# jabirali/bodge

Measured on AMD Instinct MI355X. Metric: Chebyshev SpMV steps/s + achieved HBM GB/s, 4N×4N BdG H; free_energy wall-time, higher is better.
Workload: dtype f64

## Files before the change

### bodge_amd/backend.py

```python

from __future__ import annotations

import ctypes as C
import os

import numpy as np

LIBRARY_PATH = os.environ.get(
    "BODGE_AMD_LIBRARY", os.path.join(os.path.dirname(os.path.abspath(__file__)), "csrc", "libbodge_hip.so")
)

VEC_RADEMACHER = 0
VEC_Z4 = 1

_f64p = C.POINTER(C.c_double)
_i32p = C.POINTER(C.c_int32)
_i64p = C.POINTER(C.c_int64)
_u8p = C.POINTER(C.c_uint8)
_handle = C.c_void_p


class Perf(C.Structure):
    _fields_ = [
        ("kernel_ms", C.c_double),
# ... 18 lines not shown
        ("window_ms", C.c_double),
        ("sweeps", C.c_int64),
        ("persistent", C.c_int32),
        ("groups_per_launch", C.c_int32),
        ("clenshaw", C.c_int32),
        ("green", C.c_int32),
        ("green_ranges", C.c_int32),
        ("green_local", C.c_int32),
        ("apply", C.c_int32),
        ("green_states", C.c_int32),
        ("green_bonds", C.c_int32),
        ("roll_chunk", C.c_int32),
        ("response_map", C.c_int32),
        ("gemm_ms", C.c_double),
        ("gemm_flops", C.c_double),
        ("correlation", C.c_int32),
        ("gram_ms", C.c_double),
        ("gram_flops", C.c_double),
    ]


class Operator(C.Structure):

    _fields_ = [("nnzb", C.c_int32), ("indptr", _i32p), ("indices", _i32p), ("data", _f64p)]


SIGNATURES = {
    "bdg_last_error": (C.c_char_p, []),
    "bdg_version": (C.c_char_p, []),
    "bdg_device_count": (C.c_int, [C.POINTER(C.c_int)]),
# ... 167 lines not shown
```

### bodge_amd/build.py

```python

from __future__ import annotations

import os
import shutil
import subprocess
import sys

ROOT = os.path.dirname(os.path.abspath(__file__))
CSRC = os.path.join(ROOT, "csrc")
INCLUDE = os.path.join(os.path.dirname(ROOT), "include")
LIBRARY = os.path.join(CSRC, "libbodge_hip.so")
SOURCES = [os.path.join(CSRC, "bodge_hip.hip")]
HEADERS = [os.path.join(CSRC, name) for name in (
    "kernels.hpp", "sweep.hpp", "twostage.hpp", "host_assembly.hpp", "core.hpp", "plans.hpp", "libraries.hpp", "recurrence.hpp", "family.hpp", "fermi.hpp", "apply.hpp", "correlation.hpp", "response_map.hpp", "green_driver.hpp", "green.hpp", "green_map.hpp", "green_bonds.hpp", "green_states.hpp",
    "lanczos.hpp", "subspace.hpp", "dense.hpp", "tridiag.hpp", "knobs.hpp")] + [os.path.join(INCLUDE, "bodge_hip.h")]
ARCH = "gfx950"


def _hipcc() -> str:
    found = shutil.which("hipcc") or "/opt/rocm/bin/hipcc"
    if not os.path.exists(found):
        raise RuntimeError("hipcc not found; the HIP library cannot be built")
    return found


def is_stale() -> bool:
    if not os.path.exists(LIBRARY):
        return True
    built = os.path.getmtime(LIBRARY)
# ... 27 lines not shown
```

### bodge_amd/csrc/bodge_hip.hip

```cpp

#include "bodge_hip.h"

#include <dlfcn.h>
#include <fcntl.h>
#include <hip/hip_runtime.h>
#include <rccl/rccl.h>
#include <rocsolver/rocsolver.h>

#include <sys/stat.h>
#include <unistd.h>

#include <algorithm>
#include <atomic>
#include <chrono>
#include <condition_variable>
#include <cmath>
#include <cstdarg>
#include <cstdio>
#include <cstdlib>
#include <cstring>
#include <map>
#include <memory>
#include <mutex>
#include <string>
#include <string_view>
#include <thread>
#include <tuple>
#include <type_traits>
#include <unordered_map>
#include <vector>

#include "knobs.hpp"
#include "host_assembly.hpp"
#include "kernels.hpp"
#include "sweep.hpp"
#include "twostage.hpp"

#include "core.hpp"
#include "plans.hpp"
#include "libraries.hpp"
#include "recurrence.hpp"
#include "family.hpp"
#include "fermi.hpp"
#include "apply.hpp"
#include "correlation.hpp"
#include "response_map.hpp"
#include "green_driver.hpp"
#include "green.hpp"
#include "green_map.hpp"
#include "green_bonds.hpp"
// ... 48 lines not shown
                return fail(BDG_EINVAL, "column index %d out of range in row %lld", indices[k],
                            (long long)i);
            if (k > indptr[i] && indices[k] == indices[k - 1])
                return fail(BDG_EINVAL, "row %lld has a duplicate column", (long long)i);
            if (ncols == nb && k > indptr[i] && indices[k] < indices[k - 1])
                return fail(BDG_EINVAL, "row %lld is not sorted", (long long)i);
            bandwidth = std::max<int64_t>(bandwidth, std::llabs((long long)indices[k] - (long long)i));
        }
    }
    constexpr int kMaxDistinct = 256;
    constexpr unsigned kStreamedId = 0xFEu;
    int dict_skipped = 0;
    bool onsite_streamed = false, bonds_streamed = false;
    std::vector<int> ids;
    std::vector<double> distinct;
    {
        const char* env = knob::raw("BODGE_AMD_DICT");
        bool wanted = !(env && env[0] == '0') && nnzb > 0 && ncols <= (1 << 24);
        dict_skipped = (env && env[0] == '0') ? 3 : ncols > (1 << 24) ? 2 : 0;
        auto onsite_packable = [](const double* blk) {
            auto re = [&](int r, int c) { return blk[2 * (4 * r + c)]; };
            auto im = [&](int r, int c) { return blk[2 * (4 * r + c) + 1]; };
            if (im(0, 0) != 0.0 || im(1, 1) != 0.0 || re(1, 0) != re(0, 1) || im(1, 0) != -im(0, 1)) return false;
            for (int i = 0; i < 2; ++i)
                for (int j = 0; j < 2; ++j) {
                    if (re(2 + i, j) != re(j, 2 + i) || im(2 + i, j) != -im(j, 2 + i)) return false;
                    if (re(2 + i, 2 + j) != -re(i, j) || im(2 + i, 2 + j) != im(i, j)) return false;
                }
            return true;
        };
        auto dedupe = [&](bool skip_diagonal, int limit) -> bool {
            std::unordered_map<std::string_view, int> seen;
            const double* recent_key[4] = {nullptr, nullptr, nullptr, nullptr};
            int recent_id[4] = {0, 0, 0, 0};
            int recent_next = 0;
            ids.assign((size_t)nnzb, 0);
            distinct.clear();
            for (int64_t i = 0; i < nb; ++i)
                for (int64_t k = indptr[i]; k < indptr[i + 1]; ++k) {
                    const double* block = data + 32 * k;
                    if (skip_diagonal && indices[k] == i) {
                        if (!onsite_packable(block)) return false;
                        ids[(size_t)k] = (int)((unsigned)indices[k] | (kStreamedId << 24));
                        continue;
                    }
// ... 168 lines not shown
    if (!ids.empty()) {
        sys->n_unique = (int)(distinct.size() / 32);
        if (int rc = sys->dict_ids.reserve(ids.size())) return cleanup(rc);
        if (int rc = sys->dict_full.reserve((size_t)sys->n_unique * 16)) return cleanup(rc);
        std::vector<int> diagonal((size_t)sys->n_unique, 1);
        for (int d = 0; d < sys->n_unique; ++d)
            for (int e = 0; e < 16; ++e)
                if ((e >> 2) != (e & 3) && (distinct[(size_t)32 * d + 2 * e] != 0.0 || distinct[(size_t)32 * d + 2 * e + 1] != 0.0))
                    diagonal[(size_t)d] = 0;
        for (int d = 0; d < sys->n_unique; ++d) {
            if (diagonal[(size_t)d]) continue;
            auto zero = [&](int r, int c) { return distinct[(size_t)32 * d + 2 * (4 * r + c)] == 0.0 && distinct[(size_t)32 * d + 2 * (4 * r + c) + 1] == 0.0; };
            if (zero(0, 1) && zero(1, 0) && zero(0, 2) && zero(1, 3) && zero(2, 0) && zero(3, 1) && zero(2, 3) && zero(3, 2)) diagonal[(size_t)d] = 2;
        }
        if (knob::raw("BODGE_AMD_NO_DIAGONAL_BLOCKS")) std::fill(diagonal.begin(), diagonal.end(), 0);
        if (int rc = sys->dict_diagonal.reserve((size_t)sys->n_unique)) return cleanup(rc);
        if (hipMemcpy(sys->dict_diagonal.ptr, diagonal.data(), sizeof(int) * diagonal.size(), hipMemcpyHostToDevice) != hipSuccess)
            return cleanup(fail(BDG_EDEVICE, "upload of the block dictionary failed"));
        if (!onsite_streamed && max_row <= 7) {
            const int words = max_row <= 3 ? 4 : 8;
            std::vector<unsigned> ell((size_t)nb * words, 0xFFFFFFFFu);
            for (int64_t i = 0; i < nb; ++i)
                for (int64_t k = indptr[i]; k < indptr[i + 1]; ++k) ell[(size_t)i * words + (size_t)(k - indptr[i])] = (unsigned)ids[(size_t)k];
            if (int rc = sys->dict_ell.reserve(ell.size())) return cleanup(rc);
            if (hipMemcpy(sys->dict_ell.ptr, ell.data(), sizeof(unsigned) * ell.size(), hipMemcpyHostToDevice) != hipSuccess)
                return cleanup(fail(BDG_EDEVICE, "upload of the block dictionary failed"));
            sys->dict_ell_words = words;
        }
        if (hipMemcpy(sys->dict_ids.ptr, ids.data(), sizeof(int) * ids.size(), hipMemcpyHostToDevice) != hipSuccess ||
            hipMemcpy(sys->dict_full.ptr, distinct.data(), sizeof(double) * distinct.size(),
// ... 780 lines not shown
```

### bodge_amd/csrc/core.hpp

```cpp
#pragma once

namespace {

thread_local std::string g_error;

int fail(int code, const char* fmt, ...) {
    char buf[512];
    va_list ap;
    va_start(ap, fmt);
    vsnprintf(buf, sizeof buf, fmt, ap);
    va_end(ap);
    g_error = buf;
    return code;
}

#define HIP_TRY(expr)                                                                   \
    do {                                                                                \
        hipError_t err__ = (expr);                                                      \
        if (err__ != hipSuccess)                                                        \
            return fail(err__ == hipErrorOutOfMemory ? BDG_ENOMEM : BDG_EDEVICE,        \
                        "%s failed: %s (%s:%d)", #expr, hipGetErrorString(err__),       \
                        __FILE__, __LINE__);                                            \
    } while (0)

// ... 138 lines not shown
    int dict_skipped = 0;
    bool onsite_streamed = false;
    DeviceBuffer<double2> onsite[2];
    bool bonds_streamed = false;
    DeviceBuffer<double2> site_records[2];
    int site_records_plane[2] = {0, 0};
    DeviceBuffer<int> dict_ids;
    DeviceBuffer<unsigned> dict_ell;
    int dict_ell_words = 0;
    DeviceBuffer<int> dict_diagonal;
    DeviceBuffer<double2> dict_full;
    DeviceBuffer<double2> dict_table[4];
    DeviceBuffer<uint2> stencil;
    int stencil_state = 0;
    bool stencil_wrap_p = false, stencil_wrap_x = false;
    double* host_dots = nullptr;
    size_t host_dots_count = 0;
    int shape[3] = {0, 0, 0};
    struct TileOrder {
        int rows_per_tile = 0, strip_rows = 0;
        DeviceBuffer<int> ids;
    };
    std::vector<std::unique_ptr<TileOrder>> tile_orders;
    bdg_perf perf{};
};

namespace {
inline void release_side_sets(bdg_system* sys) {
    for (auto& side : sys->side_sets) {
        if (side->stream) (void)hipStreamSynchronize(side->stream);
// ... 20 lines not shown
```

### bodge_amd/csrc/plans.hpp

```cpp
#pragma once

namespace {

using StepKernel = void (*)(bdg::StepArgs);

using bdg::ComplexMode;
using bdg::ComplexPHMode;
using bdg::RealMode;
using bdg::RealPHMode;

struct ModeInfo {
    int id;
    bool real, ph;
    int per_lane;
    int stride;
    double block_bytes;
    double entry_bytes;
};

ModeInfo mode_info(bool real, bool ph) {
    if (real && ph) return {3, true, true, RealPHMode::kVec, RealPHMode::kBlockStride, 100.0, 96.0};
    if (real) return {1, true, false, RealMode::kVec, RealMode::kBlockStride, 132.0, 96.0};
    if (ph) return {2, false, true, ComplexPHMode::kVec, ComplexPHMode::kBlockStride, 196.0, 192.0};
    return {0, false, false, ComplexMode::kVec, ComplexMode::kBlockStride, 260.0, 192.0};
// ... 441 lines not shown
        const int resident = waves * (int)std::min<size_t>(waves > 4 ? 1 : 2, sys->lds_per_cu / lds);
        if (resident > best_resident) best = waves, best_resident = resident;
    }
    return best;
}

SweepKernel sweep3_kernel(const ModeInfo& mode, int lanes, bool reverse) {
    switch (mode.id) {
        case 1: return sweep3_kernel_for<RealMode>(lanes, reverse);
        case 2: return sweep3_kernel_for<ComplexPHMode>(lanes, reverse);
        case 3: return sweep3_kernel_for<RealPHMode>(lanes, reverse);
    }
    return sweep3_kernel_for<ComplexMode>(lanes, reverse);
}

using MarchKernel = void (*)(bdg::MarchArgs);
template <typename Mode>
MarchKernel march3_kernel_for(int lanes) {
    switch (lanes) {
        case 2: return bdg::cheb_march3<Mode, 2, 0>;
        case 4: return bdg::cheb_march3<Mode, 4, 0>;
    }
    return nullptr;
}
MarchKernel march3_kernel(const ModeInfo& mode, int lanes, bool streamed, bool bonds) {
    if (streamed) {
        if (!mode.ph || lanes != 4) return nullptr;
        if (bonds) return mode.real ? bdg::cheb_march3<RealPHMode, 4, 2> : nullptr;
        return mode.real ? bdg::cheb_march3<RealPHMode, 4, 1> : bdg::cheb_march3<ComplexPHMode, 4, 1>;
    }
    switch (mode.id) {
        case 1: return march3_kernel_for<RealMode>(lanes);
        case 2: return march3_kernel_for<ComplexPHMode>(lanes);
        case 3: return march3_kernel_for<RealPHMode>(lanes);
    }
    return march3_kernel_for<ComplexMode>(lanes);
}

struct SweepPlan {
    int lanes = bdg::kSweepLanes;
    int depth = 2;
    SweepKernel kernel = nullptr, kernel_reverse = nullptr;
    SweepKernel kernel_gen = nullptr;
    MarchKernel march = nullptr;
    int march_grid = 0;
    int grid = 0;
    int wg_waves = bdg::kSweepWaves;
    size_t lds_bytes = 0;
    bdg::SweepArgs args{};
    int waves = 0;
    int whole_segs = 1;
    int segments_for(int planes) const {
        if (planes >= args.lx) return whole_segs;
        return std::max(1, std::min(choose_segments(args.n_cols, planes, waves, 2 * depth, 2), planes / 2));
    }
};

constexpr int64_t kSweepMinSites = 150000;
// ... 20 lines not shown
                if (x == 0 && (lo < 0 || lo == base)) lo = base;
                else if (x == lx - 1 && (hi < 0 || hi == base)) hi = base;
                else slab_ok = false;
            }
            for (int64_t base : {lo, hi})
                if (base >= 0 && (base < sys->nb || base + plane > sys->ncols)) slab_ok = false;
            if (slab_ok) {
                sys->stencil_lo_base = (int)lo;
                sys->stencil_hi_base = (int)hi;
            }
        }
        if (shaped && slab_ok && sys->n_unique > 0 && sys->n_unique < (int)bdg::kNoBlock &&
            sys->max_row_blocks <= (three_d ? 7 : 5) && sys->nnzb > 0 && !(three_d && sys->onsite_streamed)) {
            if (int rc = sys->stencil.reserve((size_t)sys->nb)) return rc;
            DeviceBuffer<int> bad;
            if (int rc = bad.reserve(3)) return rc;
            int host_bad[3] = {1, 0, 0};
            auto body = [&]() -> int {
                HIP_TRY(hipMemsetAsync(bad.ptr, 0, 3 * sizeof(int), sys->stream));
                const unsigned grid = (unsigned)std::min<int64_t>(4096, (sys->nb + 255) / 256);
                if (three_d)
                    bdg::build_stencil3<<<grid, 256, 0, sys->stream>>>(sys->indptr.ptr, sys->dict_ids.ptr,
                                                                        sys->dict_diagonal.ptr, (int)sys->nb, (int)plane,
                                                                        sys->shape[2], sys->stencil_lo_base, sys->stencil_hi_base,
                                                                        sys->stencil.ptr, bad.ptr);
                else
                    bdg::build_stencil<<<grid, 256, 0, sys->stream>>>(sys->indptr.ptr, sys->dict_ids.ptr,
                                                                       sys->dict_diagonal.ptr, (int)sys->nb, (int)plane,
                                                                       sys->bonds_streamed ? 2 : sys->onsite_streamed ? 1 : 0,
                                                                       sys->stencil.ptr, bad.ptr);
                HIP_TRY(hipGetLastError());
                HIP_TRY(hipMemcpyAsync(host_bad, bad.ptr, 3 * sizeof(int), hipMemcpyDeviceToHost, sys->stream));
                HIP_TRY(hipStreamSynchronize(sys->stream));
                return BDG_OK;
            };
            const int rc = body();
            bad.release();
            if (rc) return rc;
            if (host_bad[0] == 0) {
                sys->stencil_state = three_d ? 2 : 1;
                sys->stencil_wrap_p = host_bad[1] != 0;
                sys->stencil_wrap_x = host_bad[2] != 0;
            } else {
                sys->stencil.release();
            }
        }
    }
    *kind = std::max(0, sys->stencil_state);
    return BDG_OK;
}

inline int64_t plane_sites(const bdg_system* sys) { return (int64_t)sys->shape[1] * sys->shape[2]; }

int sweep_wanted(bdg_system* sys, bool col_scalars, int* kind, bool wide_call = false) {
    *kind = 0;
    const char* env = knob::raw("BODGE_AMD_SWEEP");
    if ((env && env[0] == '0') || col_scalars) return BDG_OK;
// ... 20 lines not shown
        return fail(BDG_EINVAL, "streamed on-site blocks need the three-step sweep, particle-hole packed blocks and a lane count whose ring of records fits the LDS (%d lanes do not)", lanes);
    plan->wg_waves = wg_waves;
    plan->kernel = streamed ? sweep3_streamed_kernel(mode, lanes, wg_waves, false, false, bonds)
                            : depth == 3 ? sweep3_kernel(mode, lanes, false) : sweep_kernel(mode, lanes, false);
    plan->kernel_reverse = streamed ? sweep3_streamed_kernel(mode, lanes, wg_waves, true, false, bonds)
                                    : depth == 3 ? sweep3_kernel(mode, lanes, true) : sweep_kernel(mode, lanes, true);
    plan->kernel_gen = streamed ? sweep3_streamed_kernel(mode, lanes, wg_waves, false, true, bonds) : depth == 3 ? sweep3_gen_kernel(mode, lanes) : nullptr;
    if (!plan->kernel) return fail(BDG_EINVAL, "the sweep kernel has 1, 2 or 4 lanes per site, not %d", lanes);
    const size_t table = (size_t)sys->n_unique * mode.stride * sizeof(double2);
    if (table > table_limit(sys)) return fail(BDG_EINVAL, "block table too large for the sweep kernel");
    if (depth == 3) {
        plan->lds_bytes = sweep3_lds_bytes(sys, mode, lanes, wg_waves);
    } else {
        plan->lds_bytes = table + (size_t)bdg::kSweepWaves * depth * bdg::kWave * 4 * sizeof(double2);
    }
    if (plan->lds_bytes > 64 * 1024)
        for (SweepKernel k : {plan->kernel, plan->kernel_reverse, plan->kernel_gen})
            if (k) HIP_TRY(hipFuncSetAttribute(reinterpret_cast<const void*>(k), hipFuncAttributeMaxDynamicSharedMemorySize,
                                        (int)plan->lds_bytes));
    plan->march = depth == 3 && wg_waves == bdg::kWavesPerBlock &&
                          (size_t)sys->ncols * lanes * 4 * sizeof(double2) < ((size_t)1 << 31) && sys->ncols == sys->nb
                      ? march3_kernel(mode, lanes, streamed, bonds) : nullptr;
    if (plan->march && plan->lds_bytes > 64 * 1024)
        HIP_TRY(hipFuncSetAttribute(reinterpret_cast<const void*>(plan->march), hipFuncAttributeMaxDynamicSharedMemorySize,
                                    (int)plan->lds_bytes));
    int per_cu = 0;
    HIP_TRY(hipOccupancyMaxActiveBlocksPerMultiprocessor(&per_cu, reinterpret_cast<const void*>(plan->kernel),
                                                         wg_waves * bdg::kWave, plan->lds_bytes));
    per_cu = std::max(1, std::min(per_cu, wg_waves > 4 ? 1 : 2 * bdg::kWavesPerBlock / bdg::kSweepWaves));
    if (const char* cap = knob::raw("BODGE_AMD_BLOCKS_PER_CU")) per_cu = std::max(1, atoi(cap));
    const int64_t plane = (int64_t)sys->shape[1] * sys->shape[2];
    bdg::SweepArgs& a = plan->args;
// ... 12 lines not shown
    const int owned = depth == 3 ? bdg::sweep3_owned(lanes) : bdg::sweep_owned(lanes);
    a.n_cols = (int)((plane + owned - 1) / owned);
    if (const char* env = knob::raw("BODGE_AMD_STREAMED_SHARE"); streamed && (wg_waves > 4 || (env && env[0] == '0'))) share = 1;
    const int waves = std::max(wg_waves, per_cu * sys->num_cus * wg_waves / std::max(1, share));
    int n_segs = choose_segments(a.n_cols, a.lx, waves, 2 * depth, 8, share > 1 ? 0.985 : 0.97);
    if (const char* env = knob::raw("BODGE_AMD_SWEEP_SEGMENTS")) n_segs = atoi(env);
    a.n_segs = std::max(1, std::min(n_segs, a.lx / 8));
    a.x_lo = 0;
    a.x_hi = a.lx;
    plan->waves = waves;
    plan->whole_segs = a.n_segs;
    a.zigzag = 1;
    if (const char* env = knob::raw("BODGE_AMD_SWEEP_ZIGZAG")) a.zigzag = atoi(env) != 0;
    a.wrap_p = sys->stencil_wrap_p ? 1 : 0;
    a.wrap_x = sys->stencil_wrap_x ? 1 : 0;
    const int64_t units = (int64_t)a.n_cols * a.n_segs;
    const int grid = (int)std::min<int64_t>((int64_t)per_cu * sys->num_cus, (units + wg_waves - 1) / wg_waves);
    plan->grid = std::max(8, (grid + 7) / 8 * 8);
    const int march_grid = (int)std::min<int64_t>((int64_t)per_cu * sys->num_cus,
                                                  (units * std::max(1, share) + wg_waves - 1) / wg_waves);
    plan->march_grid = std::max(8, (march_grid + 7) / 8 * 8);
    return BDG_OK;
}

double sweep_bytes(const bdg_system* sys, const ModeInfo& mode, int lanes) {
    const double onsite = !sys->onsite_streamed ? 0.0
                          : sys->bonds_streamed ? (mode.real ? 128.0 : 224.0)
                          : 16.0 * (mode.real ? RealPHMode::kOnsiteSlots : ComplexPHMode::kOnsiteSlots);
    return (8.0 + onsite) * (double)sys->nb + (mode.block_bytes - 4.0) * sys->n_unique +
           4.0 * (4.0 * lanes * sizeof(double2)) * (double)sys->nb;
// ... 165 lines not shown
```

### bodge_amd/csrc/recurrence.hpp

```cpp
#pragma once

namespace {

constexpr int kMarchAborted = -77;

struct Batch {
    bdg_system* sys = nullptr;
    StreamSet* ss = nullptr;
    int next = 0;
    int stream_share = 1;
    StepPlan plan;
    bdg::StepArgs args{};
    bool real = false;
    bool alternate = false;
    int64_t band_lo = -1, band_hi = -1;
    int plane_lo = -1, plane_hi = -1;
    ModeInfo mode{};
    int rl = 0, rv = 0, n_active = 0, n_steps = 0, chunk = 1, strip_rows = 0;
    size_t width = 0, per_step = 0, vec_count = 0;
    double scale = 1.0;
    double2* cur = nullptr;
    double2* prev = nullptr;
    float kernel_ms = 0.f;
    int n_chunks = 0;
    bool sweep = false, roll = false;
    bool gen_start = false;
    int slot = 0, n_slots = 1, ev_base = 0;
    size_t host_stride = 0;
    SweepPlan splan;
    RollPlan rplan;
    double2 *spare1 = nullptr, *spare2 = nullptr;
    const double2 *ext_lo = nullptr, *ext_hi = nullptr;
    int64_t ext_lo_site0 = 0, ext_lo_ld = 0, ext_hi_site0 = 0, ext_hi_ld = 0;
    int launch_grid = 0;
    bool discard_last = true;
    double bytes_moved = 0.0;
    bool march = false, march_follower = false;
    int march_levels = 0;
    bool march_fixed = false;
    int n_sweeps = 0;
    int64_t sweeps_counted = 0;
    hipStream_t work_stream = nullptr;
    double vector_bytes() const { return 4.0 * rl * sizeof(double2) * (double)sys->nb; }
    int n_launches = 0;

    int begin(bdg_system* system, double scale_in, int steps, int active, const StartSpec& start,
              int force_real , bool col_scalars = false, int set_index = 0) {
        sys = system;
        scale = scale_in;
        n_steps = steps;
        n_active = active;
// ... 61 lines not shown
            if (int rc = make_sweep_plan(sys, mode, rl, sweep_depth_for(sys, rl), &splan, stream_share)) return rc;
        } else if (roll) {
            plan = StepPlan{};
            plan.rl = rl;
            plan.mode = mode;
            plan.dictionary = true;
            args = bdg::StepArgs{};
            if (int rc = make_roll_plan(sys, mode, rl, &rplan)) return rc;
            rplan.share = stream_share;
        } else {
            if (int rc = make_plan(sys, rl, mode, &plan, col_scalars)) return rc;
            if (int rc = matrix_args(sys, plan, &args)) return rc;
        }
        launch_grid = sweep ? splan.grid : roll ? rplan.grid : plan.grid;
        n_launches = 0;
        n_sweeps = 0;
        sweeps_counted = 0;
        bytes_moved = 0.0;
        work_stream = ss->stream;
        march_follower = false;
        march = sweep && splan.depth == 3 && splan.march != nullptr && !sys->march_off && n_steps >= 4 &&
                start.kind == StartKind::Random;
        march_levels = 0;
        march_fixed = false;
        {
            const char* env = knob::raw("BODGE_AMD_MARCH");
            const int kind = env ? atoi(env) : 0;
            march = march && kind >= 1 && kind <= 3;
            march_levels = kind == 2 ? 1 : 0;
            march_fixed = kind == 3;
// ... 359 lines not shown
        }
        if (in_chunk == 0) HIP_TRY(hipEventRecord(ss->ev_pool[2 * (ev_base + chunk_id)], st));
        bdg::SweepArgs& a = splan.args;
        a.cur = cur;
        a.prev = n == 0 ? nullptr : prev;
        a.out1 = spare1;
        a.out2 = spare2;
        a.coef1 = (n == 0 ? 1.0 : 2.0) / scale;
        a.coef2 = 2.0 / scale;
        a.two = now >= 2 ? 1 : 0;
        a.steps = now;
        a.discard = discard_last && n + now == n_steps;
        a.partial1 = ss->partial.ptr + (size_t)in_chunk * per_step;
        a.partial2 = a.partial1 + per_step;
        a.partial3 = a.partial2 + per_step;
        const SweepKernel kernel = n == 0 && gen_start ? splan.kernel_gen
                                   : alternate && (n_launches & 1) ? splan.kernel_reverse : splan.kernel;
        if (n == 0 && gen_start) a.cur = nullptr;
        a.x_lo = 0;
        a.x_hi = a.lx;
        if (plane_lo >= 0) {
            a.x_lo = std::max(0, plane_lo - (n + now));
            a.x_hi = std::min(a.lx, plane_hi + n + now + 1);
        }
        a.n_segs = splan.segments_for(a.x_hi - a.x_lo);
        bytes_moved += (sweep_bytes(sys, mode, rl) -
                        vector_bytes() * ((n == 0 ? 1 : 0) + (n == 0 && gen_start ? 1 : 0) + (a.discard ? 2 : now == 1 ? 1 : 0))) *
                       ((double)(a.x_hi - a.x_lo) / a.lx);
        kernel<<<splan.grid, splan.wg_waves * bdg::kWave, splan.lds_bytes, st>>>(a);
        ++n_launches;
        double2* old_cur = cur;
        double2* old_prev = prev;
// ... 80 lines not shown
            for (int r = 0; r < n_active; ++r) {
                double& d = d_out[(size_t)n * ld + col0 + r];
                double& e = e_out[(size_t)n * ld + col0 + r];
                const double dv = host[(size_t)n * width + 2 * r], ev = host[(size_t)n * width + 2 * r + 1];
                d = accumulate ? d + dv : dv;
                e = accumulate ? e + ev : ev;
            }
        bdg_perf& p = sys->perf;
        if (first_batch) p = bdg_perf{};
        p.kernel_ms += kernel_ms;
        p.launches += sweep ? n_launches : n_steps;
        p.bytes_moved += bytes_moved;
        p.window_ms = p.kernel_ms;
        p.streams = 1;
        p.vector_steps += (int64_t)n_steps * n_active;
        p.bytes_per_launch = sweep  ? sweep_bytes(sys, mode, rl)
                             : roll ? roll_bytes(sys, mode, rl)
                                    : algorithmic_bytes(sys, rv, mode, plan.dictionary);
        p.steps_per_launch = sweep ? splan.depth : 1;
        p.persistent = march ? 1 : 0;
        p.sweeps += march ? sweeps_counted : sweep ? n_launches : 0;
        p.rolling = roll ? 1 : 0;
        p.roll_chunk = roll ? rplan.args.chunk : 0;
        p.dict_skipped = sys->dict_skipped;
        p.onsite_streamed = sweep && sys->onsite_streamed ? (sys->bonds_streamed ? 2 : 1) : 0;
        p.lanes_per_row = rl;
        p.vectors_per_launch = rv;
        p.real_arithmetic = real ? 1 : 0;
        p.ph_packed = mode.ph ? 1 : 0;
        p.dict_blocks = plan.dictionary ? sys->n_unique : 0;
// ... 464 lines not shown
```

### bodge_amd/csrc/sweep.hpp

```cpp
#pragma once

#include "kernels.hpp"

namespace bdg {

constexpr int kSweepLanes = 4;
constexpr int kSweepSlots = kWave / kSweepLanes;
constexpr int kSweepOwned = kSweepSlots - 4;
constexpr int sweep_owned(int rl) { return kWave / rl - 4; }
constexpr unsigned kNoBlock = 0xFFu;

struct SweepArgs {
    const uint2* stencil;
    const void* dict_table;
    int n_unique;
    const double2* onsite;
    const double2* cur;
    const double2* prev;
    double2* out1;
    double2* out2;
    double* partial1;
    double* partial2;
    double coef1, coef2;
    int nb;
// ... 1 lines not shown
    int lx;
    int n_cols;
    int n_segs;
    int two;
    int steps;
    double* partial3;
    int stream;
    int zigzag;
    int wrap_p;
    int wrap_x;
    uint64_t gen_seed, gen_first_id;
    int gen_kind;
    int gen_active;
    int discard;
    int x_lo, x_hi;
};

__global__ void build_stencil(const int* __restrict__ indptr, const int* __restrict__ words,
                              const int* __restrict__ diagonal, int nb, int plane, int onsite_streamed,
                              uint2* __restrict__ stencil, int* __restrict__ bad) {
    const int lx = nb / plane;
    for (int i = blockIdx.x * blockDim.x + threadIdx.x; i < nb; i += gridDim.x * blockDim.x) {
        unsigned id[5] = {kNoBlock, kNoBlock, kNoBlock, kNoBlock, kNoBlock};
        unsigned mask = 0;
        const int p = i % plane, x = i / plane;
        bool ok = true;
        for (int k = indptr[i]; k < indptr[i + 1]; ++k) {
            const unsigned w = (unsigned)words[k];
            const int off = (int)(w & 0xFFFFFFu) - i;
            int slot = -1;
// ... 1202 lines not shown
```

### include/bodge_hip.h

```cpp
#ifndef BODGE_HIP_H
#define BODGE_HIP_H

#include <stdint.h>

#ifdef __cplusplus
extern "C" {
#endif

#define BDG_OK 0
#define BDG_EINVAL (-1)
#define BDG_EDEVICE (-2)
#define BDG_ENOMEM (-3)
#define BDG_ELIBRARY (-4)

#define BDG_VEC_RADEMACHER 0
#define BDG_VEC_Z4 1

typedef struct bdg_system bdg_system;
typedef struct bdg_comm bdg_comm;
typedef struct bdg_group bdg_group;

typedef struct bdg_perf {
    double kernel_ms;
    int64_t launches;
// ... 17 lines not shown
    double window_ms;
    int64_t sweeps;
    int32_t persistent;
    int32_t groups_per_launch;
    int32_t clenshaw;
    int32_t green;
    int32_t green_ranges;
    int32_t green_local;
    int32_t apply;
    int32_t green_states;
    int32_t green_bonds;
    int32_t roll_chunk;
    int32_t response_map;
    double gemm_ms;
    double gemm_flops;
    int32_t correlation;
    double gram_ms;
    double gram_flops;
} bdg_perf;

const char* bdg_last_error(void);
const char* bdg_version(void);

int bdg_device_count(int* count);

int bdg_create(int device, int64_t nb, int64_t nnzb, const int32_t* indptr,
               const int32_t* indices, const double* data, bdg_system** out);
int bdg_destroy(bdg_system* sys);

int bdg_create_slab(int device, int64_t nb, int64_t ncols, int64_t nnzb, const int32_t* indptr,
// ... 122 lines not shown
```

Before: 110,600.

## Add translation-invariant sweep kernel holding stencil blocks in registers

Adds a classification pass that detects when every site in a 2D lattice uses the same bond and onsite blocks with no wrap-around. For that case it selects a specialised depth-3 sweep kernel that loads the five blocks once into registers instead of reading a per-site stencil and dictionary entries. The goal is to remove the per-site stencil reads and table lookups from the memory-bound Chebyshev SpMV. The cost is an extra classification kernel at setup and more register pressure, and the fast path applies only to uniform lattices.

```diff
diff --git a/bodge_amd/backend.py b/bodge_amd/backend.py
--- a/bodge_amd/backend.py
+++ b/bodge_amd/backend.py
@@ -56,6 +56,7 @@
         ("response_map", C.c_int32),
         ("gemm_ms", C.c_double),
         ("gemm_flops", C.c_double),
+        ("plain_stencil", C.c_int32),
         ("correlation", C.c_int32),
         ("gram_ms", C.c_double),
         ("gram_flops", C.c_double),
diff --git a/bodge_amd/build.py b/bodge_amd/build.py
--- a/bodge_amd/build.py
+++ b/bodge_amd/build.py
@@ -12,7 +12,7 @@
 LIBRARY = os.path.join(CSRC, "libbodge_hip.so")
 SOURCES = [os.path.join(CSRC, "bodge_hip.hip")]
 HEADERS = [os.path.join(CSRC, name) for name in (
-    "kernels.hpp", "sweep.hpp", "twostage.hpp", "host_assembly.hpp", "core.hpp", "plans.hpp", "libraries.hpp", "recurrence.hpp", "family.hpp", "fermi.hpp", "apply.hpp", "correlation.hpp", "response_map.hpp", "green_driver.hpp", "green.hpp", "green_map.hpp", "green_bonds.hpp", "green_states.hpp",
+    "kernels.hpp", "sweep.hpp", "sweep_plain.hpp", "twostage.hpp", "host_assembly.hpp", "core.hpp", "plans.hpp", "libraries.hpp", "recurrence.hpp", "family.hpp", "fermi.hpp", "apply.hpp", "correlation.hpp", "response_map.hpp", "green_driver.hpp", "green.hpp", "green_map.hpp", "green_bonds.hpp", "green_states.hpp",
     "lanczos.hpp", "subspace.hpp", "dense.hpp", "tridiag.hpp", "knobs.hpp")] + [os.path.join(INCLUDE, "bodge_hip.h")]
 ARCH = "gfx950"
 
diff --git a/bodge_amd/csrc/bodge_hip.hip b/bodge_amd/csrc/bodge_hip.hip
--- a/bodge_amd/csrc/bodge_hip.hip
+++ b/bodge_amd/csrc/bodge_hip.hip
@@ -34,6 +34,7 @@
 #include "host_assembly.hpp"
 #include "kernels.hpp"
 #include "sweep.hpp"
+#include "sweep_plain.hpp"
 #include "twostage.hpp"
 
 #include "core.hpp"
@@ -112,21 +113,21 @@
     bool onsite_streamed = false, bonds_streamed = false;
     std::vector<int> ids;
     std::vector<double> distinct;
+    auto onsite_packable = [](const double* blk) {
+        auto re = [&](int r, int c) { return blk[2 * (4 * r + c)]; };
+        auto im = [&](int r, int c) { return blk[2 * (4 * r + c) + 1]; };
+        if (im(0, 0) != 0.0 || im(1, 1) != 0.0 || re(1, 0) != re(0, 1) || im(1, 0) != -im(0, 1)) return false;
+        for (int i = 0; i < 2; ++i)
+            for (int j = 0; j < 2; ++j) {
+                if (re(2 + i, j) != re(j, 2 + i) || im(2 + i, j) != -im(j, 2 + i)) return false;
+                if (re(2 + i, 2 + j) != -re(i, j) || im(2 + i, 2 + j) != im(i, j)) return false;
+            }
+        return true;
+    };
     {
         const char* env = knob::raw("BODGE_AMD_DICT");
         bool wanted = !(env && env[0] == '0') && nnzb > 0 && ncols <= (1 << 24);
         dict_skipped = (env && env[0] == '0') ? 3 : ncols > (1 << 24) ? 2 : 0;
-        auto onsite_packable = [](const double* blk) {
-            auto re = [&](int r, int c) { return blk[2 * (4 * r + c)]; };
-            auto im = [&](int r, int c) { return blk[2 * (4 * r + c) + 1]; };
-            if (im(0, 0) != 0.0 || im(1, 1) != 0.0 || re(1, 0) != re(0, 1) || im(1, 0) != -im(0, 1)) return false;
-            for (int i = 0; i < 2; ++i)
-                for (int j = 0; j < 2; ++j) {
-                    if (re(2 + i, j) != re(j, 2 + i) || im(2 + i, j) != -im(j, 2 + i)) return false;
-                    if (re(2 + i, 2 + j) != -re(i, j) || im(2 + i, 2 + j) != im(i, j)) return false;
-                }
-            return true;
-        };
         auto dedupe = [&](bool skip_diagonal, int limit) -> bool {
             std::unordered_map<std::string_view, int> seen;
             const double* recent_key[4] = {nullptr, nullptr, nullptr, nullptr};
@@ -325,6 +326,8 @@
             if (zero(0, 1) && zero(1, 0) && zero(0, 2) && zero(1, 3) && zero(2, 0) && zero(3, 1) && zero(2, 3) && zero(3, 2)) diagonal[(size_t)d] = 2;
         }
         if (knob::raw("BODGE_AMD_NO_DIAGONAL_BLOCKS")) std::fill(diagonal.begin(), diagonal.end(), 0);
+        sys->dict_packable.resize((size_t)sys->n_unique);
+        for (int d = 0; d < sys->n_unique; ++d) sys->dict_packable[(size_t)d] = onsite_packable(distinct.data() + (size_t)32 * d) ? 1 : 0;
         if (int rc = sys->dict_diagonal.reserve((size_t)sys->n_unique)) return cleanup(rc);
         if (hipMemcpy(sys->dict_diagonal.ptr, diagonal.data(), sizeof(int) * diagonal.size(), hipMemcpyHostToDevice) != hipSuccess)
             return cleanup(fail(BDG_EDEVICE, "upload of the block dictionary failed"));
diff --git a/bodge_amd/csrc/core.hpp b/bodge_amd/csrc/core.hpp
--- a/bodge_amd/csrc/core.hpp
+++ b/bodge_amd/csrc/core.hpp
@@ -176,6 +176,10 @@
     DeviceBuffer<uint2> stencil;
     int stencil_state = 0;
     bool stencil_wrap_p = false, stencil_wrap_x = false;
+    bool plain_stencil = false;
+    unsigned plain_ids = 0, plain_meta = 0;
+    int plain_onsite_form = 0;
+    std::vector<unsigned char> dict_packable;
     double* host_dots = nullptr;
     size_t host_dots_count = 0;
     int shape[3] = {0, 0, 0};
diff --git a/bodge_amd/csrc/plans.hpp b/bodge_amd/csrc/plans.hpp
--- a/bodge_amd/csrc/plans.hpp
+++ b/bodge_amd/csrc/plans.hpp
@@ -479,6 +479,16 @@
     return sweep3_kernel_for<ComplexMode>(lanes, reverse);
 }
 
+constexpr bool kSweepPlainDefault = true;
+template <int OSF>
+SweepKernel sweep3_plain_pick(bool reverse, bool gen) {
+    return gen ? bdg::cheb_sweep3_plain<RealPHMode, false, true, OSF>
+               : reverse ? bdg::cheb_sweep3_plain<RealPHMode, true, false, OSF> : bdg::cheb_sweep3_plain<RealPHMode, false, false, OSF>;
+}
+SweepKernel sweep3_plain_kernel(int form, bool reverse, bool gen) {
+    return form == 1 ? sweep3_plain_pick<1>(reverse, gen) : sweep3_plain_pick<0>(reverse, gen);
+}
+
 using MarchKernel = void (*)(bdg::MarchArgs);
 template <typename Mode>
 MarchKernel march3_kernel_for(int lanes) {
@@ -507,6 +517,8 @@
     int depth = 2;
     SweepKernel kernel = nullptr, kernel_reverse = nullptr;
     SweepKernel kernel_gen = nullptr;
+    bool plain = false;
+    SweepKernel plain_kernel = nullptr, plain_reverse = nullptr, plain_gen = nullptr;
     MarchKernel march = nullptr;
     int march_grid = 0;
     int grid = 0;
@@ -557,10 +569,16 @@
             sys->max_row_blocks <= (three_d ? 7 : 5) && sys->nnzb > 0 && !(three_d && sys->onsite_streamed)) {
             if (int rc = sys->stencil.reserve((size_t)sys->nb)) return rc;
             DeviceBuffer<int> bad;
-            if (int rc = bad.reserve(3)) return rc;
-            int host_bad[3] = {1, 0, 0};
+            if (int rc = bad.reserve(3 + bdg::kPlainWords)) return rc;
+            int host_bad[3 + bdg::kPlainWords] = {1, 0, 0, 1};
+            const bool classify = !three_d && !sys->onsite_streamed && !sys->bonds_streamed;
             auto body = [&]() -> int {
-                HIP_TRY(hipMemsetAsync(bad.ptr, 0, 3 * sizeof(int), sys->stream));
+                {
+                    int init[3 + bdg::kPlainWords] = {0};
+                    for (int slot = 0; slot < 5; ++slot) init[3 + 1 + slot] = 0xFF;
+                    HIP_TRY(hipMemcpyAsync(bad.ptr, init, sizeof(init), hipMemcpyHostToDevice, sys->stream));
+                    HIP_TRY(hipStreamSynchronize(sys->stream));
+                }
                 const unsigned grid = (unsigned)std::min<int64_t>(4096, (sys->nb + 255) / 256);
                 if (three_d)
                     bdg::build_stencil3<<<grid, 256, 0, sys->stream>>>(sys->indptr.ptr, sys->dict_ids.ptr,
@@ -573,7 +591,12 @@
                                                                        sys->bonds_streamed ? 2 : sys->onsite_streamed ? 1 : 0,
                                                                        sys->stencil.ptr, bad.ptr);
                 HIP_TRY(hipGetLastError());
-                HIP_TRY(hipMemcpyAsync(host_bad, bad.ptr, 3 * sizeof(int), hipMemcpyDeviceToHost, sys->stream));
+                if (classify) {
+                    bdg::classify_stencil<<<std::min(grid, 256u), 256, 0, sys->stream>>>(sys->stencil.ptr, sys->dict_diagonal.ptr, (int)sys->nb,
+                                                                                        (int)plane, bad.ptr + 3);
+                    HIP_TRY(hipGetLastError());
+                }
+                HIP_TRY(hipMemcpyAsync(host_bad, bad.ptr, sizeof(host_bad), hipMemcpyDeviceToHost, sys->stream));
                 HIP_TRY(hipStreamSynchronize(sys->stream));
                 return BDG_OK;
             };
@@ -584,6 +607,18 @@
                 sys->stencil_state = three_d ? 2 : 1;
                 sys->stencil_wrap_p = host_bad[1] != 0;
                 sys->stencil_wrap_x = host_bad[2] != 0;
+                const int* seen = host_bad + 3;
+                bool plain = classify && !sys->stencil_wrap_p && !sys->stencil_wrap_x && seen[0] == 0;
+                for (int slot = 0; slot < 5 && plain; ++slot) plain = seen[1 + slot] == seen[6 + slot] && seen[1 + slot] < (int)bdg::kNoBlock;
+                if (plain) {
+                    const int centre = seen[1 + 2];
+                    const bool singlet = seen[11] == (1 << 2);
+                    plain = singlet || (centre < (int)sys->dict_packable.size() && sys->dict_packable[(size_t)centre]);
+                    sys->plain_onsite_form = singlet ? 1 : 0;
+                    sys->plain_ids = (unsigned)seen[1] | ((unsigned)seen[2] << 8) | ((unsigned)seen[3] << 16) | ((unsigned)seen[4] << 24);
+                    sys->plain_meta = (unsigned)seen[5];
+                }
+                sys->plain_stencil = plain;
             } else {
                 sys->stencil.release();
             }
@@ -634,8 +669,17 @@
     } else {
         plan->lds_bytes = table + (size_t)bdg::kSweepWaves * depth * bdg::kWave * 4 * sizeof(double2);
     }
+    plan->plain = false;
+    bool plain_wanted = kSweepPlainDefault;
+    if (const char* env = knob::raw("BODGE_AMD_SWEEP_PLAIN")) plain_wanted = env[0] != '0';
+    if (plain_wanted && depth == 3 && !streamed && lanes == 2 && mode.id == 3 && sys->plain_stencil) {
+        plan->plain = true;
+        plan->plain_kernel = sweep3_plain_kernel(sys->plain_onsite_form, false, false);
+        plan->plain_reverse = sweep3_plain_kernel(sys->plain_onsite_form, true, false);
+        plan->plain_gen = sweep3_plain_kernel(sys->plain_onsite_form, false, true);
+    }
     if (plan->lds_bytes > 64 * 1024)
-        for (SweepKernel k : {plan->kernel, plan->kernel_reverse, plan->kernel_gen})
+        for (SweepKernel k : {plan->kernel, plan->kernel_reverse, plan->kernel_gen, plan->plain_kernel, plan->plain_reverse, plan->plain_gen})
             if (k) HIP_TRY(hipFuncSetAttribute(reinterpret_cast<const void*>(k), hipFuncAttributeMaxDynamicSharedMemorySize,
                                         (int)plan->lds_bytes));
     plan->march = depth == 3 && wg_waves == bdg::kWavesPerBlock &&
@@ -678,6 +722,8 @@
     if (const char* env = knob::raw("BODGE_AMD_SWEEP_ZIGZAG")) a.zigzag = atoi(env) != 0;
     a.wrap_p = sys->stencil_wrap_p ? 1 : 0;
     a.wrap_x = sys->stencil_wrap_x ? 1 : 0;
+    a.plain_ids = sys->plain_ids;
+    a.plain_meta = sys->plain_meta;
     const int64_t units = (int64_t)a.n_cols * a.n_segs;
     const int grid = (int)std::min<int64_t>((int64_t)per_cu * sys->num_cus, (units + wg_waves - 1) / wg_waves);
     plan->grid = std::max(8, (grid + 7) / 8 * 8);
diff --git a/bodge_amd/csrc/recurrence.hpp b/bodge_amd/csrc/recurrence.hpp
--- a/bodge_amd/csrc/recurrence.hpp
+++ b/bodge_amd/csrc/recurrence.hpp
@@ -35,6 +35,7 @@
     int launch_grid = 0;
     bool discard_last = true;
     double bytes_moved = 0.0;
+    int plain_launches = 0;
     bool march = false, march_follower = false;
     int march_levels = 0;
     bool march_fixed = false;
@@ -126,6 +127,7 @@
         }
         launch_grid = sweep ? splan.grid : roll ? rplan.grid : plan.grid;
         n_launches = 0;
+        plain_launches = 0;
         n_sweeps = 0;
         sweeps_counted = 0;
         bytes_moved = 0.0;
@@ -515,8 +517,11 @@
         a.partial1 = ss->partial.ptr + (size_t)in_chunk * per_step;
         a.partial2 = a.partial1 + per_step;
         a.partial3 = a.partial2 + per_step;
-        const SweepKernel kernel = n == 0 && gen_start ? splan.kernel_gen
-                                   : alternate && (n_launches & 1) ? splan.kernel_reverse : splan.kernel;
+        const bool plain = splan.plain && plane_lo < 0;
+        const SweepKernel kernel = n == 0 && gen_start ? (plain ? splan.plain_gen : splan.kernel_gen)
+                                   : alternate && (n_launches & 1) ? (plain ? splan.plain_reverse : splan.kernel_reverse)
+                                                                   : (plain ? splan.plain_kernel : splan.kernel);
+        plain_launches += plain ? 1 : 0;
         if (n == 0 && gen_start) a.cur = nullptr;
         a.x_lo = 0;
         a.x_hi = a.lx;
@@ -627,6 +632,7 @@
         p.window_ms = p.kernel_ms;
         p.streams = 1;
         p.vector_steps += (int64_t)n_steps * n_active;
+        p.plain_stencil = sweep && plain_launches > 0 ? 1 : 0;
         p.bytes_per_launch = sweep  ? sweep_bytes(sys, mode, rl)
                              : roll ? roll_bytes(sys, mode, rl)
                                     : algorithmic_bytes(sys, rv, mode, plan.dictionary);
diff --git a/bodge_amd/csrc/sweep.hpp b/bodge_amd/csrc/sweep.hpp
--- a/bodge_amd/csrc/sweep.hpp
+++ b/bodge_amd/csrc/sweep.hpp
@@ -39,6 +39,7 @@
     int gen_active;
     int discard;
     int x_lo, x_hi;
+    unsigned plain_ids, plain_meta;
 };
 
 __global__ void build_stencil(const int* __restrict__ indptr, const int* __restrict__ words,
diff --git a/bodge_amd/csrc/sweep_plain.hpp b/bodge_amd/csrc/sweep_plain.hpp
--- /dev/null
+++ b/bodge_amd/csrc/sweep_plain.hpp
@@ -0,0 +1,314 @@
+#pragma once
+
+#include "sweep.hpp"
+
+namespace bdg {
+
+constexpr int kPlainWords = 12;
+
+__global__ void classify_stencil(const uint2* __restrict__ stencil, const int* __restrict__ diagonal, int nb, int plane,
+                                 int* __restrict__ out) {
+    __shared__ int red[kPlainWords];
+    if (threadIdx.x < kPlainWords) red[threadIdx.x] = threadIdx.x >= 1 && threadIdx.x <= 5 ? 0xFF : 0;
+    __syncthreads();
+    const int lx = nb / plane;
+    int bad = 0, kinds = 0, lo[5] = {0xFF, 0xFF, 0xFF, 0xFF, 0xFF}, hi[5] = {0, 0, 0, 0, 0};
+    for (int i = blockIdx.x * blockDim.x + threadIdx.x; i < nb; i += gridDim.x * blockDim.x) {
+        const uint2 w = stencil[i];
+        const int p = i % plane, x = i / plane;
+        const bool expect[5] = {x >= 1, p >= 1, true, p <= plane - 2, x <= lx - 2};
+#pragma unroll
+        for (int slot = 0; slot < 5; ++slot) {
+            const int id = (int)(slot < 4 ? (w.x >> (8 * slot)) & 0xFFu : w.y & 0xFFu);
+            const bool flagged = (w.y >> (8 + slot)) & 1u;
+            if ((id != (int)kNoBlock) != expect[slot]) bad = 1;
+            if (id == (int)kNoBlock) continue;
+            if (flagged != (slot != 2)) bad = 1;
+            lo[slot] = min(lo[slot], id);
+            hi[slot] = max(hi[slot], id);
+            if (slot == 2) kinds |= 1 << diagonal[id];
+        }
+    }
+    if (bad) atomicOr(red, 1);
+    for (int slot = 0; slot < 5; ++slot) {
+        atomicMin(red + 1 + slot, lo[slot]);
+        atomicMax(red + 6 + slot, hi[slot]);
+    }
+    atomicOr(red + 11, kinds);
+    __syncthreads();
+    if (threadIdx.x == 0) atomicOr(out, red[0]);
+    else if (threadIdx.x <= 5) atomicMin(out + threadIdx.x, red[threadIdx.x]);
+    else if (threadIdx.x <= 10) atomicMax(out + threadIdx.x, red[threadIdx.x]);
+    else if (threadIdx.x == 11) atomicOr(out + 11, red[11]);
+}
+
+typedef const double __attribute__((address_space(4)))* PlainConstDoubles;
+
+template <typename Mode>
+__device__ __forceinline__ void plain_block(const void* table, unsigned id, double2 (&blk)[Mode::kSlotsPerBlock]) {
+    const PlainConstDoubles t = (PlainConstDoubles)(uintptr_t)table + (size_t)id * Mode::kSlotsPerBlock * 2;
+#pragma unroll
+    for (int e = 0; e < Mode::kSlotsPerBlock; ++e) blk[e] = make_double2(t[2 * e], t[2 * e + 1]);
+}
+
+template <typename Mode, int OSF>
+struct PlainBlocks {
+    double2 bond[4][Mode::kDiagSlots];
+    double2 onsite[OSF == 1 ? Mode::kSingletSlots : Mode::kOnsiteSlots];
+};
+
+template <typename Mode>
+__device__ __forceinline__ void plain_onsite_record(const double2 (&blk)[Mode::kSlotsPerBlock], double2 (&rec)[Mode::kOnsiteSlots]) {
+    if constexpr (Mode::kVec == 2) {
+        rec[0] = blk[0];
+        rec[1] = make_double2(blk[1].y, 0.0);
+        rec[2] = blk[2];
+        rec[3] = blk[3];
+    } else {
+        rec[0] = make_double2(blk[0].x, blk[3].x);
+        rec[1] = blk[1];
+        rec[2] = blk[4], rec[3] = blk[5], rec[4] = blk[6], rec[5] = blk[7];
+    }
+}
+
+template <typename Mode, int OSF, bool GEN, bool RV>
+__device__ __forceinline__ void plain_unit(const SweepArgs& a, const PlainBlocks<Mode, OSF>& blocks, double2* const row_0, double2* const row_1,
+                                           double2* const row_2, const Sweep3Gen& gen, int lane, int seg, int col, double (&dot1)[4],
+                                           double (&dot2)[4], double (&dot3)[4]) {
+    constexpr int RL = 2;
+    constexpr int SLOTS = kWave / RL;
+    constexpr int OWNED3 = SLOTS - 6;
+    const int s = lane / RL;
+    const int r = lane % RL;
+    const double2 zero = make_double2(0.0, 0.0);
+    const size_t nb = (size_t)a.nb;
+    const int steps = a.steps;
+
+    const int x0 = a.x_lo + (int)(((int64_t)(a.x_hi - a.x_lo) * seg) / a.n_segs);
+    const int x1 = a.x_lo + (int)(((int64_t)(a.x_hi - a.x_lo) * (seg + 1)) / a.n_segs);
+    const int p = col * OWNED3 - 3 + s;
+    const bool inside = p >= 0 && p < a.plane;
+    const bool ok1 = inside && s >= 1 && s <= SLOTS - 2;
+    const bool ok2 = inside && s >= 2 && s <= SLOTS - 3;
+    const bool owned = inside && s >= 3 && s <= SLOTS - 4;
+    const double coef1 = ok1 ? a.coef1 : 0.0;
+    const int lane_m = s >= 1 ? lane - RL : lane, lane_p = s <= SLOTS - 2 ? lane + RL : lane;
+
+    auto act = [&](int k) { return RV ? x0 + x1 - 1 - k : k; };
+    auto in_lattice = [&](int k) { return act(k) >= 0 && act(k) < a.lx; };
+    const int plane_bytes = a.plane * RL * (int)sizeof(double2);
+    const int lane_bytes = (p * RL + r) * (int)sizeof(double2);
+    const int off_in = inside ? lane_bytes : kBufferOutOfRange;
+    const int off_ok1 = ok1 ? lane_bytes : kBufferOutOfRange;
+    const int off_owned = owned ? lane_bytes : kBufferOutOfRange;
+    auto load_plane = [&](const double2* buf, int k, int offset, double2 out[4]) {
+        k = act(k);
+        const bool there = buf != nullptr && k >= 0 && k < a.lx;
+#pragma unroll
+        for (int al = 0; al < 4; ++al) {
+            const __amdgpu_buffer_rsrc_t rsrc = sweep_plane_rsrc(buf, there ? ((size_t)al * nb + (size_t)k * a.plane) * RL * sizeof(double2) : 0,
+                                                                 there ? plane_bytes : 0);
+            out[al] = __builtin_bit_cast(double2, __builtin_amdgcn_raw_buffer_load_b128(rsrc, offset, 0, 0));
+        }
+    };
+    auto store_plane = [&](double2* buf, int k, const double2 v[4]) {
+        if (a.discard) return;
+#pragma unroll
+        for (int al = 0; al < 4; ++al) {
+            const __amdgpu_buffer_rsrc_t rsrc = sweep_plane_rsrc(buf, ((size_t)al * nb + (size_t)act(k) * a.plane) * RL * sizeof(double2), plane_bytes);
+            __builtin_amdgcn_raw_buffer_store_b128(__builtin_bit_cast(u32x4, v[al]), rsrc, off_owned, 0, 0);
+        }
+    };
+    auto cur_plane = [&](int k, bool wanted, double2 out[4]) {
+        if constexpr (GEN) {
+            k = act(k);
+            const bool there = wanted && k >= 0 && k < a.lx;
+            const uint64_t site = (uint64_t)k * a.plane + (inside ? p : 0);
+            const uint64_t h0 = start_site_hash(gen.key0, site);
+            [[maybe_unused]] const uint64_t h1 = Mode::kVec == 2 ? start_site_hash(gen.key1, site) : 0;
+#pragma unroll
+            for (int al = 0; al < 4; ++al) {
+                if constexpr (Mode::kVec == 2) {
+                    out[al].x = there && inside && gen.on0 ? start_component(h0, al, 0).x : 0.0;
+                    out[al].y = there && inside && gen.on1 ? start_component(h1, al, 0).x : 0.0;
+                } else {
+                    out[al] = there && inside && gen.on0 ? start_component(h0, al, a.gen_kind) : zero;
+                }
+            }
+        } else {
+            load_plane(a.cur, k, wanted ? off_in : kBufferOutOfRange, out);
+        }
+    };
+    auto put_own = [&](double2* row, const double2 v[4]) {
+#pragma unroll
+        for (int be = 0; be < 4; ++be) row[SHARE_SLOT(lane, be)] = v[be];
+    };
+    auto wave_order = [&]() {
+        __builtin_amdgcn_fence(__ATOMIC_ACQ_REL, "wavefront");
+        __builtin_amdgcn_wave_barrier();
+    };
+    auto apply = [&](const double2* row, const double2 before[4], const double2 after[4], double2 mid[4], double2 acc[4]) {
+        double2 xm[4], xp[4];
+#pragma unroll
+        for (int be = 0; be < 4; ++be) {
+            mid[be] = row[SHARE_SLOT(lane, be)];
+            xm[be] = row[SHARE_SLOT(lane_m, be)];
+            xp[be] = row[SHARE_SLOT(lane_p, be)];
+        }
+#pragma unroll
+        for (int al = 0; al < 4; ++al) acc[al] = zero;
+        Mode::mac_diag_compact(acc, blocks.bond[0], RV ? after : before);
+        Mode::mac_diag_compact(acc, blocks.bond[1], xm);
+        if constexpr (OSF == 1) Mode::mac_singlet(acc, blocks.onsite, mid);
+        else Mode::mac_onsite(acc, blocks.onsite, mid);
+        Mode::mac_diag_compact(acc, blocks.bond[2], xp);
+        Mode::mac_diag_compact(acc, blocks.bond[3], RV ? before : after);
+    };
+    auto dots_owned = [&](double (&dot)[4], const double2 mid[4], const double2 made[4]) {
+#pragma unroll
+        for (int al = 0; al < 4; ++al) Mode::dots(dot, owned ? mid[al] : zero, made[al]);
+    };
+
+    const int k_first = x0 - (steps - 1), k_last = x1 + steps - 2;
+
+    double2 cn_m[4], buf_a[4], buf_b[4], pv[4], c1_m[4], c2_m[4];
+    cur_plane(k_first - 1, true, cn_m);
+    cur_plane(k_first, true, buf_a);
+    cur_plane(k_first + 1, true, buf_b);
+    load_plane(GEN ? nullptr : a.prev, k_first, off_ok1, pv);
+#pragma unroll
+    for (int al = 0; al < 4; ++al) c1_m[al] = c2_m[al] = zero;
+    wave_order();
+    put_own(row_1, c1_m);
+    put_own(row_2, c1_m);
+
+    auto iterate = [&](int k, double2 (&centre)[4], const double2 (&after)[4]) {
+        const bool more = k < k_last;
+        put_own(row_0, centre);
+        wave_order();
+        cur_plane(k + 2, more, centre);
+
+        double2 new1[4], new2[4], mid1[4], mid2[4];
+#pragma unroll
+        for (int al = 0; al < 4; ++al) new1[al] = new2[al] = zero;
+        {
+            double2 acc[4], mid0[4];
+            apply(row_0, cn_m, after, mid0, acc);
+            if (in_lattice(k)) {
+#pragma unroll
+                for (int al = 0; al < 4; ++al) {
+                    new1[al].x = fma(coef1, acc[al].x, -pv[al].x);
+                    new1[al].y = fma(coef1, acc[al].y, -pv[al].y);
+                }
+                if (k >= x0 && k < x1) {
+                    dots_owned(dot1, mid0, new1);
+                    if (steps == 1) store_plane(a.out2, k, new1);
+                    if (steps == 2) store_plane(a.out1, k, new1);
+                }
+            }
+        }
+        load_plane(GEN ? nullptr : a.prev, k + 1, more ? off_ok1 : kBufferOutOfRange, pv);
+
+        {
+            double2 acc[4];
+            apply(row_1, c1_m, new1, mid1, acc);
+            wave_order();
+            put_own(row_1, new1);
+            if (steps >= 2 && in_lattice(k - 1) && k - 1 >= x0 - (steps - 2) && k - 1 < x1 + (steps - 2)) {
+#pragma unroll
+                for (int al = 0; al < 4; ++al) {
+                    new2[al].x = ok2 ? fma(a.coef2, acc[al].x, -cn_m[al].x) : 0.0;
+                    new2[al].y = ok2 ? fma(a.coef2, acc[al].y, -cn_m[al].y) : 0.0;
+                }
+                if (k - 1 >= x0 && k - 1 < x1) {
+                    dots_owned(dot2, mid1, new2);
+                    if (steps == 2) store_plane(a.out2, k - 1, new2);
+                    if (steps == 3) store_plane(a.out1, k - 1, new2);
+                }
+            }
+        }
+
+        {
+            double2 acc[4];
+            apply(row_2, c2_m, new2, mid2, acc);
+#pragma unroll
+            for (int be = 0; be < 4; ++be) cn_m[be] = row_0[SHARE_SLOT(lane, be)];
+            wave_order();
+            put_own(row_2, new2);
+            if (steps >= 3 && k - 2 >= x0 && k - 2 < x1) {
+                double2 new3[4];
+#pragma unroll
+                for (int al = 0; al < 4; ++al) {
+                    new3[al].x = fma(a.coef2, acc[al].x, -c1_m[al].x);
+                    new3[al].y = fma(a.coef2, acc[al].y, -c1_m[al].y);
+                }
+                dots_owned(dot3, mid2, new3);
+                store_plane(a.out2, k - 2, new3);
+            }
+        }
+
+#pragma unroll
+        for (int al = 0; al < 4; ++al) {
+            c1_m[al] = mid1[al];
+            c2_m[al] = mid2[al];
+        }
+    };
+    for (int k = k_first; k <= k_last; k += 2) {
+        iterate(k, buf_a, buf_b);
+        if (k + 1 <= k_last) iterate(k + 1, buf_b, buf_a);
+    }
+}
+
+template <typename Mode, bool REV, bool GEN, int OSF = 0>
+__global__ __launch_bounds__(kBlockThreads, 2) void cheb_sweep3_plain(SweepArgs a) {
+    extern __shared__ double2 lds[];
+    constexpr int RL = 2;
+    const int lane = threadIdx.x & (kWave - 1);
+    const int wave = __builtin_amdgcn_readfirstlane(threadIdx.x / kWave);
+    const Sweep3Lds w = sweep3_stage_lds<Mode, 0, kBlockThreads>(lds, a, kWave / RL, wave);
+
+    PlainBlocks<Mode, OSF> blocks;
+    {
+        double2 blk[Mode::kSlotsPerBlock];
+#pragma unroll
+        for (int b = 0; b < 4; ++b) {
+            const int slot = b < 2 ? b : b + 1;
+            plain_block<Mode>(a.dict_table, slot < 4 ? (a.plain_ids >> (8 * slot)) & 0xFFu : a.plain_meta & 0xFFu, blk);
+            Mode::pack_diag(blocks.bond[b], blk);
+        }
+        plain_block<Mode>(a.dict_table, (a.plain_ids >> 16) & 0xFFu, blk);
+        if constexpr (OSF == 1) Mode::pack_singlet(blocks.onsite, blk);
+        else plain_onsite_record<Mode>(blk, blocks.onsite);
+    }
+
+    const int n_units = a.n_cols * a.n_segs;
+    const int xcd = blockIdx.x & 7;
+    const int u_lo = (int)(((int64_t)n_units * xcd) >> 3);
+    const int u_hi = (int)(((int64_t)n_units * (xcd + 1)) >> 3);
+    const int waves_per_xcd = (gridDim.x >> 3) * kWavesPerBlock;
+
+    double dot1[4] = {0.0, 0.0, 0.0, 0.0}, dot2[4] = {0.0, 0.0, 0.0, 0.0}, dot3[4] = {0.0, 0.0, 0.0, 0.0};
+    Sweep3Gen gen;
+    if constexpr (GEN) gen = sweep3_gen_keys<Mode>(a.gen_seed, a.gen_first_id, a.gen_active, lane % RL);
+
+    for (int u = u_lo + (int)(blockIdx.x >> 3) * kWavesPerBlock + wave; u < u_hi; u += waves_per_xcd) {
+        const int seg = u / a.n_cols, col = u - seg * a.n_cols;
+        const bool rev = REV != (bool)(a.zigzag & seg & 1);
+        if (rev) plain_unit<Mode, OSF, GEN, true>(a, blocks, w.row_0, w.row_1, w.row_2, gen, lane, seg, col, dot1, dot2, dot3);
+        else plain_unit<Mode, OSF, GEN, false>(a, blocks, w.row_0, w.row_1, w.row_2, gen, lane, seg, col, dot1, dot2, dot3);
+    }
+
+    const int steps = a.steps;
+    __syncthreads();
+    sweep_reduce_dots<Mode, RL, kWavesPerBlock>(dot1, reinterpret_cast<double*>(lds), a.partial1, lane, wave);
+    if (steps >= 2) {
+        __syncthreads();
+        sweep_reduce_dots<Mode, RL, kWavesPerBlock>(dot2, reinterpret_cast<double*>(lds), a.partial2, lane, wave);
+    }
+    if (steps >= 3) {
+        __syncthreads();
+        sweep_reduce_dots<Mode, RL, kWavesPerBlock>(dot3, reinterpret_cast<double*>(lds), a.partial3, lane, wave);
+    }
+}
+
+}
diff --git a/include/bodge_hip.h b/include/bodge_hip.h
--- a/include/bodge_hip.h
+++ b/include/bodge_hip.h
@@ -55,6 +55,7 @@
     int32_t response_map;
     double gemm_ms;
     double gemm_flops;
+    int32_t plain_stencil;
     int32_t correlation;
     double gram_ms;
     double gram_flops;
```

New measurement: 112,200, median of 6. +1.4%, better.
